# mythos-bio/mythos

Measured on AMD Instinct MI355X. Metric: MD steps/sec (and ns/day) per GPU, oxDNA2 12 kbp duplex, higher is better.
Workload: dtype f32; 1 GPU; oxDNA2 12000 bp duplex (24000 nt), Debye-Hueckel salt 0.5, Langevin dt 0.005, free space, 1 replica/GPU; half_charged_ends=True, replicas=1, repeats=1, warmup_steps_done=10405, precision=headline f32 (north_star: fp32 at 1e-3); the other precision: --full, full=False

## Files before the change

include/mythos_hip.h:

```cpp
#ifndef MYTHOS_HIP_H
#define MYTHOS_HIP_H

#include <stdint.h>

#ifdef __cplusplus
extern "C" {
#endif

typedef struct mythos_system mythos_system_t;
typedef struct mythos_sim mythos_sim_t;
typedef struct mythos_martini mythos_martini_t;
typedef struct mythos_martini_sim mythos_martini_sim_t;
typedef struct mythos_obs mythos_obs_t;
typedef void* mythos_stream_t;

enum mythos_status {
  MYTHOS_OK = 0,
  MYTHOS_ERR_INVALID_ARGUMENT = -1,
  MYTHOS_ERR_HIP = -2,
  MYTHOS_ERR_NO_DEVICE = -3,
  MYTHOS_ERR_NOT_READY = -4,
  MYTHOS_ERR_OVERFLOW = -5,
  MYTHOS_ERR_NUMERIC = -6
};
// ... 107 lines not shown
int mythos_langevin_set_option(mythos_sim_t* sim, int option, int64_t value);

int mythos_langevin_set_timing(mythos_sim_t* sim, int samples);
int mythos_langevin_last_kernel_ms(const mythos_sim_t* sim, double* kernel_ms, double* loop_ms_per_launch,
                                   int* launches, int* samples);

int mythos_langevin_last_recoveries(const mythos_sim_t* sim, int* recoveries);
int mythos_langevin_last_rebuilds(const mythos_sim_t* sim, int* scheduled);

int mythos_umbrella_check(int n, int n_rep, int model, int n_bonded, const int32_t* bonded, int n_ops, const int32_t* op_kind,
                          const int32_t* op_first, const int32_t* pairs, int n_pairs, const int32_t* iface_first,
                          const double* interfaces, const int32_t* table_shape, const double* table, int segment_steps);
int mythos_langevin_set_umbrella(mythos_sim_t* sim, int n_rep, int n_ops, const int32_t* op_kind, const int32_t* op_first,
                                 const int32_t* pairs, int n_pairs, const int32_t* iface_first, const double* interfaces,
                                 const int32_t* table_shape, const double* table, double hb_cutoff, int segment_steps);
int mythos_langevin_advance_umbrella(mythos_sim_t* sim, int n_segments, int sample_every, void* traj_center, void* traj_quat,
                                     void* prop_center, void* prop_quat, double* record, mythos_stream_t stream);
int mythos_langevin_umbrella_counts(mythos_sim_t* sim, int64_t* accepted, int64_t* decided);

int mythos_oxdna_read_trajectory(const char* path, int n, int max_frames, double* times, double* box, double* energies,
                                 double* frames, int* n_frames);

int mythos_oxdna_write_trajectory(const char* path, int n, int n_frames, const double* times, const double* box,
                                  const double* energies, const double* frames, int append);

enum mythos_debug_key {
  MYTHOS_DEBUG_CELL_BUCKET_CAP = 0,
  MYTHOS_DEBUG_ENERGY_LIST_CAP = 1,
  MYTHOS_DEBUG_MD_SEGMENT = 2,
  MYTHOS_DEBUG_MD_OVERFLOW_AT = 3,
  MYTHOS_DEBUG_MD_DENSE = 4,
  MYTHOS_DEBUG_MD_ITEMS_BIG = 5,
  MYTHOS_DEBUG_MD_LANES = 6,
  MYTHOS_DEBUG_KEYS = 7
};
int mythos_debug_set(int key, int64_t value);
int64_t mythos_debug_get(int key);

#define MYTHOS_MARTINI_N_TERMS 3
mythos_martini_t* mythos_martini_create(int n, const int32_t* types, int n_types, const double* sigma,
                                        const double* eps, int n_bonds, const int32_t* bonds, const double* bond_k,
                                        const double* bond_r0, int n_angles, const int32_t* angles,
                                        const double* angle_k, const double* angle_t0, int angle_kind, double r_cut,
                                        int dtype, int device);
void mythos_martini_destroy(mythos_martini_t* m);
int mythos_martini_set_params(mythos_martini_t* m, const double* sigma, const double* eps, const double* bond_k, const double* bond_r0,
                              const double* angle_k, const double* angle_t0);
int mythos_martini_energy(mythos_martini_t* m, const void* pos, const void* box, int n_frames, double* e_terms,
                          void* dU_dpos, mythos_stream_t stream);

int mythos_martini_param_grads(mythos_martini_t* m, const void* pos, const void* box, int n_frames, double* d_sigma,
                               double* d_eps, double* d_bond_k, double* d_bond_r0, double* d_angle_k,
                               double* d_angle_t0, mythos_stream_t stream);

int mythos_martini_set_charges(mythos_martini_t* m, const double* q, double epsilon_r, double epsilon_rf);
int mythos_martini_coulomb(mythos_martini_t* m, const void* pos, const void* box, int n_frames, double* e_coul,
                           void* dU_dpos, mythos_stream_t stream);

mythos_martini_sim_t* mythos_martini_langevin_create(mythos_martini_t* sys, double dt, double kT, double gamma,
                                                     const double* mass, uint64_t seed);
void mythos_martini_langevin_destroy(mythos_martini_sim_t* sim);
int mythos_martini_langevin_set_neighbor_policy(mythos_martini_sim_t* sim, double skin, int rebuild_every);
int mythos_martini_langevin_set_inner_list(mythos_martini_sim_t* sim, double margin, int every);
int mythos_martini_langevin_init_velocities(mythos_martini_sim_t* sim, void* vel, mythos_stream_t stream);
int mythos_martini_langevin_run(mythos_martini_sim_t* sim, void* pos, void* vel, const double* box, int n_steps,
                                int save_every, void* traj_pos, double* e_trace, mythos_stream_t stream);
int mythos_martini_langevin_load(mythos_martini_sim_t* sim, const void* pos, const void* vel, const double* box,
// ... 99 lines not shown
```

mythos_amd/_lib.py:

```python

from __future__ import annotations

import ctypes as C
import os
from pathlib import Path

import torch

_LIB_PATH = Path(__file__).resolve().parent / "lib" / "libmythos_hip.so"

c_int_p = C.POINTER(C.c_int32)
c_double_p = C.POINTER(C.c_double)
c_uint8_p = C.POINTER(C.c_uint8)


class MythosHipError(RuntimeError):
    """An error reported by libmythos_hip.so."""


_lib = None

V = C.c_void_p
_SIGS = {
    "mythos_version": (C.c_char_p, []),
# ... 139 lines not shown
            f"{path} not found: the HIP extension is not built (run __graft_entry__.build()). "
            "mythos_amd has no CPU fallback."
        )
    lib = C.CDLL(str(path))
    for name, (res, args) in _SIGS.items():
        fn = getattr(lib, name)
        fn.restype = res
        fn.argtypes = args
    _lib = lib
    return lib


DECLARED_SYMBOLS = tuple(_SIGS)


MEMBRANE_ROW = 7


def last_error() -> str:
    return load().mythos_last_error().decode()


def check(rc: int, what: str = "") -> None:
    if rc == 0:
        return
    msg = f"{what}: {last_error()} (status {rc})"
    if rc == -1:
        raise ValueError(msg)
    if rc == -6:
        raise FloatingPointError(msg)
    raise MythosHipError(msg)


DEBUG_KEYS = {"cell_bucket_cap": 0, "energy_list_cap": 1, "md_segment": 2, "md_overflow_at": 3, "md_dense": 4, "md_items_big": 5, "md_lanes": 6}


def debug_set(key: str, value: int) -> None:
    check(load().mythos_debug_set(DEBUG_KEYS[key], int(value)), f"debug_set({key})")


def debug_get(key: str) -> int:
    return int(load().mythos_debug_get(DEBUG_KEYS[key]))


_PARAM_NAMES: list[str] = []


def param_names() -> list[str]:
    if not _PARAM_NAMES:
        lib = load()
        _PARAM_NAMES.extend(lib.mythos_oxdna_param_name(i).decode() for i in range(lib.mythos_oxdna_param_count()))
    return list(_PARAM_NAMES)


def device_count() -> int:
    return int(load().mythos_device_count())


def ptr(t):
    if t is None:
        return None
    if hasattr(t, "data_ptr"):
        return C.c_void_p(t.data_ptr())
    return C.c_void_p(t.ctypes.data)


def stream(device) -> C.c_void_p:
# ... 41 lines not shown
```

mythos_amd/csrc/capi.hip:

```cpp
#include <atomic>
#include <cmath>
#include <cstring>
#include <memory>

#include "cell_list.h"
#include "observables.h"

namespace mythos {

static thread_local std::string g_last_error;

void set_error(const std::string& msg) { g_last_error = msg; }

int hip_fail(hipError_t e, const char* what) {
  g_last_error = std::string("HIP error: ") + hipGetErrorString(e) + " in " + what;
  return MYTHOS_ERR_HIP;
}

static std::atomic<long long> g_debug[MYTHOS_DEBUG_KEYS];

long long debug_value(int key) { return (key >= 0 && key < MYTHOS_DEBUG_KEYS) ? g_debug[key].load(std::memory_order_relaxed) : 0; }
void debug_clear(int key) {
  if (key >= 0 && key < MYTHOS_DEBUG_KEYS) g_debug[key].store(0, std::memory_order_relaxed);
}

static const char* const kParamNames[] = {
#define OXP(name) #name,
#include "oxdna_param_list.inc"
#undef OXP
};

}

using namespace mythos;

extern "C" {

const char* mythos_version(void) { return "mythos_amd 0.1 (gfx950)"; }

const char* mythos_last_error(void) { return g_last_error.c_str(); }

int mythos_device_count(void) {
  int n = 0;
  if (hipGetDeviceCount(&n) != hipSuccess) return 0;
  return n;
}

int mythos_debug_set(int key, int64_t value) {
  if (key < 0 || key >= MYTHOS_DEBUG_KEYS || value < 0) {
    set_error("mythos_debug_set: unknown key or negative value");
    return MYTHOS_ERR_INVALID_ARGUMENT;
  }
// ... 315 lines not shown
```

mythos_amd/csrc/langevin.hip:

```cpp
#include <algorithm>
#include <memory>
#include <vector>

#include "langevin_core.inc"
#include "point_force_checks.h"

namespace {
MdEntries md_entries_of(const mythos_sim* s) { return s->sys->dtype == MYTHOS_F32 ? md_entries<float>() : md_entries_f64(); }

ExtFieldView ext_point_part(const ExtFieldView& v) {
  ExtFieldView o;
  o.n_points = v.n_points;
  o.pt_kind = v.pt_kind, o.pt_particle = v.pt_particle, o.pt_ref = v.pt_ref, o.pt_flags = v.pt_flags, o.pt_param = v.pt_param;
  for (int a = 0; a < 3; ++a) o.box[a] = v.box[a];
  return o;
}

int ext_entries_merge(mythos_sim* s) {
  const std::vector<int>&ri = s->h_rst_index, &rf = s->h_rst_first, &rt = s->h_rst_term, &pp = s->h_pt_particle;
  ExtFieldView& v = s->rst;
  v.n_entries = v.n_points = 0;
  v.e_index = v.e_first = v.e_term = v.pt_first = nullptr;
  std::vector<int> e_index, e_first{0}, e_term, pt_first{0};
  size_t a = 0, b = 0;
// ... 37 lines not shown
  s->device = sys->device;
  s->dt = dt;
  s->kT = kT;
  s->gamma_t = gamma_t;
  s->gamma_r = gamma_r;
  s->mass = mass;
  for (int k = 0; k < 3; ++k) s->inertia[k] = inertia ? inertia[k] : 1.0;
  s->seed = seed;
  const size_t v4 = (sys->dtype == MYTHOS_F32 ? sizeof(float4) : sizeof(double4)) * (size_t)sys->n;
  bool ok = md_run_create(*s);
  for (int k = 0; k < 2; ++k)
    for (int a = 0; a < mythos_sim::kFrameArrays; ++a) ok = ok && s->frame[k][a].alloc(v4) == 0;
  ok = ok && s->keep_hi.alloc(v4) == 0 && s->keep_lo.alloc(v4) == 0 &&
       s->d_epart.alloc((size_t)((sys->n + 15) / 16) * kTraceWidth) == 0 && sys->reserve_refs() == 0;
  if (!ok) {
    set_error("mythos_langevin_create: device allocation failed");
    return nullptr;
  }
  return s.release();
}

void mythos_langevin_destroy(mythos_sim_t* s) { delete s; }

int mythos_langevin_set_neighbor_policy(mythos_sim_t* s, double r_cut, double skin, int every) {
  if (!s || (every > 0 && (!(r_cut > 0) || !(skin > 0)))) {
    set_error("mythos_langevin_set_neighbor_policy: invalid argument");
    return MYTHOS_ERR_INVALID_ARGUMENT;
  }
  s->r_cut = r_cut;
  s->skin = skin;
  s->rebuild_every = every;
  s->list_fitted = false;
  s->list_valid = false;
  return MYTHOS_OK;
}

int mythos_langevin_init_momenta(mythos_sim_t* s, void* p_lin, void* p_ang, mythos_stream_t stream) {
  if (!s || !p_lin || !p_ang) {
    set_error("mythos_langevin_init_momenta: invalid argument");
    return MYTHOS_ERR_INVALID_ARGUMENT;
  }
  MYTHOS_HIP_TRY(hipSetDevice(s->device));
  return md_entries_of(s).init_momenta(s, p_lin, p_ang, (hipStream_t)stream);
}

namespace {

int md_ready_state(mythos_sim_t* s, const char* who) {
  mythos_system* sys = s->sys;
  if (!sys->params_set) {
    set_error(std::string(who) + ": parameters must be set first");
    return MYTHOS_ERR_NOT_READY;
  }
  if (sys->model == 4 && !sys->types_set) {
    set_error(std::string(who) + ": an oxNA system needs its nucleotide types (mythos_oxdna_set_nucleotide_types)");
    return MYTHOS_ERR_NOT_READY;
  }
  MYTHOS_HIP_TRY(hipSetDevice(sys->device));
  return MYTHOS_OK;
}

int md_ready(mythos_sim_t* s, const char* who) {
  mythos_system* sys = s->sys;
  if (int rc = md_ready_state(s, who)) return rc;
  if (!sys->nbrs_set && s->rebuild_every <= 0) {
    set_error(std::string(who) + ": parameters and neighbours (or a neighbour policy) must be set first");
// ... 553 lines not shown
```

mythos_amd/csrc/langevin_core.inc:

```
#include <algorithm>
#include <cmath>
#include <type_traits>

#include <hip/hip_ext.h>

#ifndef MYTHOS_LEAN_MATH
#define MYTHOS_LEAN_MATH 1
#endif

#include "cell_list.h"
#include "chunk_order.h"
#include "md_driver.h"
#include "md_plan.h"
#include "oxdna_gather.h"
#include "philox.h"

#include "langevin_step.h"
#include "langevin_frame.h"
#include "ext_field.h"
#include "langevin_unfused.inc"

using namespace mythos;

namespace mythos {
// ... 126 lines not shown
                               (const int*)sim->d_flags.get(), (const int*)halt_words, k, stamp, sim->d_rst_stamp.get(), st);
    }
    auto launch = [&](auto save_tag, auto items_tag, auto pseq_tag, auto dense_tag, auto lanes_tag) {
      hipExtLaunchKernelGGL((md_step_kernel<R, MODEL, decltype(save_tag)::value, decltype(items_tag)::value, decltype(pseq_tag)::value,
                                            decltype(dense_tag)::value, decltype(lanes_tag)::value>),
                            dim3(plan.grid), dim3(kMdBlock), 0, st, row.ea, row.eb, 0,
                            Pdev, box, K, cut, n, fr[cur], fr[cur ^ 1], sys->list.d_rows.get(), sys->d_row_len.get(), row_close_of(sys),
                            sys->list.stride, sys->extra_bonds ? 1 : 0, kick_close, row.do_step, sim->seed, (uint64_t)(sim->step + k), ref,
                            ref_off, ref_a1, sim->d_flags.get(), tc, tq, sim->d_epart.get(), sim->d_chunk_order.get(), halt_words, k, 0,
                            plan.prio_on, pseq);
    };
    with_bool(save, [&](auto save_tag) {
      with_bool(sim->items_big, [&](auto big_tag) {
        constexpr bool SV = decltype(save_tag)::value;
        using Items = std::integral_constant<int, decltype(big_tag)::value ? md_items_big<R, SV>() : kMdItems>;
        with_bool(use_pseq, [&](auto pseq_tag) {
          using L8 = std::integral_constant<int, 8>;
          using L16 = std::integral_constant<int, 16>;
          constexpr bool dense_exists = sizeof(R) == 4 && !SV && !decltype(pseq_tag)::value && Items::value == kMdItems && MODEL <= 2;
          if (sim->lanes == 16) {
            launch(save_tag, Items{}, pseq_tag, std::false_type{}, L16{});
          } else if constexpr (dense_exists) {
            with_bool(plan.dense_grid, [&](auto dense_tag) { launch(save_tag, Items{}, pseq_tag, dense_tag, L8{}); });
          } else {
            launch(save_tag, Items{}, pseq_tag, std::false_type{}, L8{});
          }
        });
      });
    });
    if (save)
      hipLaunchKernelGGL(reduce_trace_kernel<kTraceWidth>, dim3(1), dim3(256), 0, st, sim->d_epart.get(), blocks,
                         e_trace + (size_t)row.sidx * kTraceWidth);
  };
  auto rebuild = [&](int buf) -> int {
    if ((++sim->builds & 63) == 0)
      if (int rc = update_chunk_order<R>(sim, fr[buf].p0, blocks, st)) return rc;
    return rows_build_device(sys, fr[buf].p0, true, sim->r_cut, sim->skin, fr[buf].p3, fr[buf].p1, true, st);
  };
  auto rebuild_until_fit = [&](int buf) -> int {
    return rows_build_until_fit(sys, fr[buf].p0, true, sim->r_cut, sim->skin, fr[buf].p3, fr[buf].p1, true, true, st);
  };
  auto on_abort = [&]() -> int {
    if (!sim->items_big) {
      sim->items_big = true;
      return 0;
    }
    set_error("mythos_langevin_run: more than " + std::to_string(md_items_big<R, false>()) + " (" + std::to_string(md_items_big<R, true>()) +
              " on steps that save energies)"
              " neighbours of one nucleotide are inside the range of an angular term (overlapping bases?)");
    return MYTHOS_ERR_OVERFLOW;
  };
  MdDrive d;
  d.who = "mythos_langevin_run";
  d.n_steps = n_steps, d.save_every = save_every, d.close = close;
  d.energy_rows = save_every > 0 && e_trace != nullptr;
  d.plain_rows = save_every > 0 && e_trace == nullptr && (traj_center != nullptr || traj_quat != nullptr);
  d.dynamic_list = dynamic_list;
  d.halt_words = halt_words;
  d.row_stride = &sys->list.stride;
  d.skin = sim->skin;
  d.st = st;
  return md_drive(*sim, d, launch_step, rebuild, rebuild_until_fit, on_abort);
}

template <typename R>
static int entry_load(mythos_sim* s, void* c, void* q, void* p, void* l, hipStream_t st) {
  if (s->unfused.active) return unfused_load<R>(s, (R*)c, (R*)q, (R*)p, (R*)l, st);
  return with_model(s->sys->model, [&](auto m) { return load_typed<R, decltype(m)::value>(s, (R*)c, (R*)q, (R*)p, (R*)l, st); });
}

template <typename R>
static int entry_advance(mythos_sim* s, int n_steps, int save_every, bool close, void* tc, void* tq, double* e_trace, hipStream_t st) {
// ... 71 lines not shown
```

mythos_amd/csrc/langevin_sim.h:

```cpp
#pragma once
#ifndef MYTHOS_UNFUSED_STATE_DEFINED
#error "langevin_sim.h needs UnfusedState: include langevin_unfused.inc (or langevin_core.inc), which defines it and then includes this file"
#endif
#include <cmath>
#include <vector>

#include "ext_field.h"
#include "langevin_step.h"
#include "md_driver.h"
#include "umbrella.h"

struct mythos_sim : mythos::MdRun {
  mythos_system* sys = nullptr;
  int device = 0;
  double dt = 0, kT = 0, gamma_t = 0, gamma_r = 0, mass = 1, inertia[3] = {1, 1, 1};
  double r_cut = 0, skin = 0;
  static constexpr int kFrameArrays = 8;
  mythos::DeviceBytes frame[2][kFrameArrays];
  int builds = 0;
  int list_epoch = 0;
  mythos::DeviceBytes keep_hi, keep_lo;
  bool keep_valid = false;
  bool items_big = false;
  int param_epoch = 0;
  int lanes = mythos::kMdG;
  mythos::DeviceBuf<int> d_chunk_order;
  mythos::DeviceBuf<unsigned long long> d_chunk_keys;
  mythos::DeviceBuf<double> d_epart;
  mythos::UnfusedState unfused;
  int ext_count = 0;
  mythos::DeviceBuf<int> d_ext_index;
  mythos::DeviceBytes d_ext_force;
  mythos::DeviceBuf<unsigned long long> d_ext_stamp;
  bool ext_stamp_stale = true;
  mythos::ExtFieldView rst;
  mythos::DeviceBuf<int> d_rst_t_index, d_rst_t_mask, d_rst_g_kind, d_rst_g_first, d_rst_g_member, d_rst_g_mask;
  mythos::DeviceBuf<int> d_rst_e_index, d_rst_e_first, d_rst_e_term;
  mythos::DeviceBuf<double> d_rst_t_k, d_rst_t_anchor, d_rst_g_vec, d_rst_g_target, d_rst_g_row;
  mythos::DeviceBuf<unsigned long long> d_rst_stamp;
  bool rst_stamp_stale = true;
  mythos::DeviceBuf<int> d_pt_first, d_pt_kind, d_pt_particle, d_pt_ref, d_pt_flags;
  mythos::DeviceBuf<double> d_pt_param;
  std::vector<int> h_rst_index, h_rst_first{0}, h_rst_term, h_pt_particle;
  bool pt_moving = false;
  mythos::UmbrellaState umb;
  mythos::DeviceBytes d_eval_p0, d_eval_mom, d_eval_ctl;
  mythos::DeviceBuf<double> d_eval_group_row;
  ~mythos_sim() { (void)hipSetDevice(device); }
};

namespace mythos {

template <typename R>
// ... 45 lines not shown
```

mythos_amd/csrc/mythos_internal.h:

```cpp
#pragma once
#include <hip/hip_runtime.h>

#include <algorithm>
#include <cmath>
#include <cstdint>
#include <string>
#include <type_traits>
#include <vector>

#include "../../include/mythos_hip.h"
#include "device_buf.h"
#include "oxdna_math.h"

namespace mythos {

long long debug_value(int key);
void debug_clear(int key);

constexpr int ROW_ROLE_Q = 1 << 30;
constexpr int ROW_INDEX_MASK = ROW_ROLE_Q - 1;
constexpr int ROW_BONDED_SLOTS = 4;

template <typename R>
struct BoxT {
// ... 13 lines not shown
  int cell_alloc_bucket_cap = 0;
  bool cell_sites = false;
  int cell_bucket_cap;
  int cell_phase = 0;
  explicit VerletRows(int bucket_cap) : cell_bucket_cap(bucket_cap) {}
};

}

struct mythos_obs;

struct mythos_system {
  int model = 0;
  int n = 0;
  int dtype = 0;
  int device = 0;
  int n_bonded = 0;
  bool has_box = false;
  double box[3] = {0, 0, 0};

  mythos::DeviceBuf<int> d_meta;

  mythos::VerletRows list{32};
  mythos::DeviceBuf<int> d_row_len;
  bool nbrs_set = false;
  int list_epoch = 0;
  int param_epoch = 0;
  std::vector<int> h_partners;
  bool extra_bonds = false;

  mythos::DeviceBytes d_ref_pos;
  mythos::DeviceBytes d_ref_off;
  mythos::DeviceBytes d_ref_a1;
  int reserve_refs() {
    const size_t v4 = (dtype == MYTHOS_F32 ? sizeof(float4) : sizeof(double4)) * (size_t)n;
    for (mythos::DeviceBytes* b : {&d_ref_pos, &d_ref_off, &d_ref_a1})
      if (int rc = b->grow(v4)) return rc;
    return 0;
  }

  bool params_set = false;
  mythos::OxParams<float> pf;
  mythos::OxParams<double> pd;
  std::vector<double> pd_sets;
  int param_sets() const { return model == 4 ? 3 : 1; }
  bool types_set = false;
  std::vector<int> h_meta;
  mythos::DeviceBuf<float> d_pf;
  mythos::DeviceBuf<double> d_pd;

  mythos::DeviceBytes d_ps_marg;
  mythos::DeviceBuf<int> d_ps_unit;
  mythos::DeviceBytes d_ps_bp;
  int pseq_terms = 0;
  int ps_n_bp = 0;
  double* ps_gmarg = nullptr;
  double* ps_gbp = nullptr;

  mythos::DeviceBuf<double> d_epart;
  mythos::DeviceBuf<double> d_pgpart;
  mythos::DeviceBuf<double> d_sweep_consts;
  mythos::DeviceBuf<double> d_sweep_part;
  std::vector<int> h_op_list;
  mythos::DeviceBuf<int> d_op_list;

  ~mythos_system() { (void)hipSetDevice(device); }
// ... 57 lines not shown
  return sys->param_sets() == 1 ? sys->pd.v : sys->pd_sets.data() + (size_t)k * OXP_COUNT;
}
inline double oxdna_param_max(const mythos_system* sys, int idx) {
  double m = oxdna_param_set(sys, 0)[idx];
  for (int k = 1; k < sys->param_sets(); ++k) m = std::max(m, oxdna_param_set(sys, k)[idx]);
  return m;
}

inline double oxdna_close_range(const mythos_system* sys) {
  double off_back = 0.0, off_base = 0.0, off_stack = 0.0;
  for (int k = 0; k < std::min(sys->param_sets(), 2); ++k) {
    const double* P = oxdna_param_set(sys, k);
    off_back = std::max(off_back, std::sqrt(P[GEO_BACK_A1] * P[GEO_BACK_A1] + (sys->model >= 2 ? P[GEO_BACK_A2] * P[GEO_BACK_A2] : 0.0)));
    off_base = std::max(off_base, std::fabs(P[GEO_BASE]));
    off_stack = std::max(off_stack, std::fabs(P[GEO_STACK]));
  }
  auto mx = [&](int idx) { return oxdna_param_max(sys, idx); };
  double rcom = std::max(mx(NEXC_BACK_BASE_RC), mx(NEXC_BASE_BACK_RC)) + off_back + off_base;
  rcom = std::max(rcom, mx(NEXC_BASE_RC) + 2 * off_base);
  rcom = std::max(rcom, std::max(mx(HYDR_RCHIGH), mx(CRST_RCHIGH)) + 2 * off_base);
  rcom = std::max(rcom, mx(CXST_RCHIGH) + 2 * off_stack);
  return rcom * (1.0 + 1e-6);
}

int oxdna_energy_launch(mythos_system* sys, const void* center, const void* quat, int n_frames, double* e_terms,
                        void* dU_dcenter, void* dU_dquat, double* dU_dparams, mythos_obs* obs, double* obs_out,
                        hipStream_t stream);
int rows_from_pairs(mythos_system* sys, const int32_t* pairs, int n_pairs);
int rows_build_device(mythos_system* sys, const void* center, bool center_is_vec4, double r_cut, double skin,
                      const void* backbone_offsets, const void* base_vectors, bool write_refs, hipStream_t stream);
int rows_build_until_fit(mythos_system* sys, const void* center, bool center_is_vec4, double r_cut, double skin,
                         const void* backbone_offsets, const void* base_vectors, bool write_refs, bool headroom,
                         hipStream_t stream);

}
```

mythos_amd/csrc/neighbors.hip:

```cpp
#include <algorithm>
#include <cmath>

#include "cell_list.h"
#include "oxdna_gather.h"

namespace mythos {

int rows_from_pairs(mythos_system* sys, const int32_t* pairs, int n_pairs) {
  const int n = sys->n;
  std::vector<int> count(n, 0);
  for (int k = 0; k < n_pairs; ++k) {
    const int i = pairs[2 * k], j = pairs[2 * k + 1];
    if (i < 0 || j < 0 || i >= n || j >= n || i == j) {
      set_error("set_neighbors: pair index out of range or i == j");
      return MYTHOS_ERR_INVALID_ARGUMENT;
    }
    ++count[i];
    ++count[j];
  }
  int mx = 0;
  for (int c : count) mx = std::max(mx, c);
  const int stride = ((mx + ROW_BONDED_SLOTS + 15) / 16) * 16;
  std::vector<int> rows((size_t)n * stride, -1), len(n, ROW_BONDED_SLOTS);
  for (int i = 0; i < n; ++i) {
    for (int k = 0; k < ROW_BONDED_SLOTS; ++k) rows[(size_t)i * stride + k] = sys->h_partners[(size_t)ROW_BONDED_SLOTS * i + k];
  }
  for (int k = 0; k < n_pairs; ++k) {
    const int i = pairs[2 * k], j = pairs[2 * k + 1];
    rows[(size_t)i * stride + len[i]++] = j;
    rows[(size_t)j * stride + len[j]++] = i | ROW_ROLE_Q;
  }
  if (int rc = rows_reserve(sys->list, n, stride)) return rc;
  MYTHOS_HIP_TRY(hipMemcpy(sys->list.d_rows.get(), rows.data(), rows.size() * sizeof(int), hipMemcpyHostToDevice));
  MYTHOS_HIP_TRY(hipMemcpy(sys->d_row_len.get(), len.data(), n * sizeof(int), hipMemcpyHostToDevice));
  MYTHOS_HIP_TRY(hipMemcpy(row_close_of(sys), len.data(), n * sizeof(int), hipMemcpyHostToDevice));
  sys->nbrs_set = true;
  return 0;
// ... 207 lines not shown
      if (k < kSegCap) s_far[k] = e;
    }
    out_c += __popc(mc);
    out_f += __popc(mf);
  }
  __builtin_amdgcn_wave_barrier();
  __builtin_amdgcn_fence(__ATOMIC_ACQ_REL, "wavefront");
  const int n_close = ROW_BONDED_SLOTS + out_c;
  int out = n_close + out_f;
  group_sort_to_row<G>(s_close, min(out_c, kSegCap), row + ROW_BONDED_SLOTS, row_stride - ROW_BONDED_SLOTS, l);
  if (n_close < row_stride) group_sort_to_row<G>(s_far, min(out_f, kSegCap), row + n_close, row_stride - n_close, l);
  if (l == 0) {
    row[0] = bp.x, row[1] = bp.y, row[2] = bp.z, row[3] = bp.w;
    if (out > row_stride) {
      atomicMax(overflow, out);
      out = row_stride;
    }
    row_len[i] = out;
    row_close[i] = min(n_close, out);
    if (ref_pos) {
      R* rp = ref_pos + 4 * (size_t)i;
      rp[0] = ci.x, rp[1] = ci.y, rp[2] = ci.z, rp[3] = VEC4 ? pos[S * i + 3] : R(0);
      if (sc.off) {
        R* ro = ref_off + 4 * (size_t)i;
        R* ra = ref_a1 + 4 * (size_t)i;
#pragma unroll
        for (int k = 0; k < 4; ++k) ro[k] = sc.off[4 * (size_t)i + k], ra[k] = sc.a1[4 * (size_t)i + k];
      }
    }
  }
}

template <typename R>
static int build_cells_typed(mythos_system* sys, const R* pos, bool vec4, double rl, double skin, const R* off,
                             const R* a1, bool write_refs, hipStream_t st) {
  R* ref_pos = write_refs ? (R*)sys->d_ref_pos.get() : nullptr;
  R* ref_off = write_refs ? (R*)sys->d_ref_off.get() : nullptr;
  R* ref_a1 = write_refs ? (R*)sys->d_ref_a1.get() : nullptr;
  const int n = sys->n;
  const double rcl = sys->params_set ? std::min(rl, oxdna_close_range(sys) + skin) : rl;
  int* d_close = row_close_of(sys);
  double rbb = rl;
  if (off && sys->params_set) {
    rbb = oxdna_param_max(sys, NEXC_BACKBONE_RC);
    if (sys->model >= 2) rbb = std::max(rbb, oxdna_param_max(sys, DH_RCUT));
    rbb = std::min(rl, rbb + skin);
  }
  if (!sys->params_set || !a1) off = nullptr;
  SiteCrit<R> sc{off, a1, R(rbb * rbb), R(0), R(0), R(0), R(0), R(0)};
  if (off) {
    auto mx = [&](int idx) { return oxdna_param_max(sys, idx); };
    const double* Pd = oxdna_param_set(sys, 0);
    const double* Pr = oxdna_param_set(sys, sys->param_sets() == 1 ? 0 : 1);
    const double slack_ba = std::fabs(Pd[GEO_BASE] - Pr[GEO_BASE]), slack_st = std::fabs(Pd[GEO_STACK] - Pr[GEO_STACK]);
    auto sq = [&](double r) { return R((r + skin) * (r + skin)); };
    sc.rbase2 = sq(std::max({mx(HYDR_RCHIGH), mx(CRST_RCHIGH), mx(NEXC_BASE_RC)}) + slack_ba);
    sc.rstack2 = sq(mx(CXST_RCHIGH) + slack_st);
    sc.rkb2 = sq(std::max(mx(NEXC_BACK_BASE_RC), mx(NEXC_BASE_BACK_RC)) + 0.5 * slack_ba);
    sc.g_ba = R(0.5 * (Pd[GEO_BASE] + Pr[GEO_BASE]));
    sc.g_st = R(0.5 * (Pd[GEO_STACK] + Pr[GEO_STACK]));
  }
  VerletRows& L = sys->list;
  CellGrid<R> g;
  const bool cells = cell_grid(g, n, rl, sys->has_box ? sys->box : nullptr);
  const int blocks_ap = (n * 64 + 255) / 256;
  int* d_partners = sys->d_row_len.get() + n;
  const BoxT<R> box = make_box<R>(sys);
  if (!cells) {
    if (vec4)
      hipLaunchKernelGGL((build_rows_allpairs_kernel<R, true>), dim3(blocks_ap), dim3(256), 0, st, n, pos, box,
                         R(rl * rl), R(rcl * rcl), sc, d_partners, L.d_rows.get(), sys->d_row_len.get(), d_close, L.stride, L.d_overflow.get());
    else
      hipLaunchKernelGGL((build_rows_allpairs_kernel<R, false>), dim3(blocks_ap), dim3(256), 0, st, n, pos, box,
                         R(rl * rl), R(rcl * rcl), sc, d_partners, L.d_rows.get(), sys->d_row_len.get(), d_close, L.stride, L.d_overflow.get());
    if (write_refs && vec4) {
      const size_t bytes = (size_t)n * 4 * sizeof(R);
      MYTHOS_HIP_TRY(hipMemcpyAsync(ref_pos, pos, bytes, hipMemcpyDeviceToDevice, st));
      if (sc.off) {
        MYTHOS_HIP_TRY(hipMemcpyAsync(ref_off, sc.off, bytes, hipMemcpyDeviceToDevice, st));
        MYTHOS_HIP_TRY(hipMemcpyAsync(ref_a1, sc.a1, bytes, hipMemcpyDeviceToDevice, st));
      }
    }
    return 0;
  }
  const bool sites = sc.off != nullptr && vec4;
  CellBins bins;
  if (int rc = cell_table<R>(L, next_pow2(2 * n), sites, st, bins)) return rc;
  const size_t site_stride = sites ? (size_t)bins.H * bins.cap : 0;
  if (vec4)
    cell_bins_build<R, true>(n, pos, g, bins, L.d_overflow.get(), false, st, sc.off, sc.a1);
  else
    cell_bins_build<R, false>(n, pos, g, bins, L.d_overflow.get(), false, st);
  constexpr int kPerBlock = 256 / kRowG;
  const int wb = (n + kPerBlock - 1) / kPerBlock;
  const size_t far_lds = (size_t)kPerBlock * 2 * L.stride * sizeof(int);
  if (vec4)
    hipLaunchKernelGGL((build_rows_cells_kernel<R, true, kRowG>), dim3(wb), dim3(256), far_lds, st, n, pos, box, g, R(rl * rl),
                       R(rcl * rcl), sc, d_partners, bins.cnt_cur, (const typename CellPlace<R>::type*)bins.place, bins.cap, bins.spill, bins.H, site_stride, L.d_rows.get(), sys->d_row_len.get(), d_close, L.stride,
                       L.d_overflow.get(), ref_pos, ref_off, ref_a1);
  else
    hipLaunchKernelGGL((build_rows_cells_kernel<R, false, kRowG>), dim3(wb), dim3(256), far_lds, st, n, pos, box, g, R(rl * rl),
                       R(rcl * rcl), sc, d_partners, bins.cnt_cur, (const typename CellPlace<R>::type*)bins.place, bins.cap, bins.spill, bins.H, site_stride, L.d_rows.get(), sys->d_row_len.get(), d_close, L.stride,
                       L.d_overflow.get(), ref_pos, ref_off, ref_a1);
  return 0;
}

int rows_build_device(mythos_system* sys, const void* center, bool center_is_vec4, double r_cut, double skin,
                      const void* backbone_offsets, const void* base_vectors, bool write_refs, hipStream_t stream) {
  if (sys->list.stride == 0)
    if (int rc = rows_reserve(sys->list, sys->n, 64)) return rc;
  const double rl = r_cut + skin;
  int rc;
  if (sys->dtype == MYTHOS_F32)
    rc = build_cells_typed<float>(sys, (const float*)center, center_is_vec4, rl, skin, (const float*)backbone_offsets, (const float*)base_vectors, write_refs, stream);
  else
    rc = build_cells_typed<double>(sys, (const double*)center, center_is_vec4, rl, skin, (const double*)backbone_offsets, (const double*)base_vectors, write_refs, stream);
  if (rc) return rc;
  MYTHOS_HIP_TRY(hipGetLastError());
  sys->nbrs_set = true;
  return 0;
}

int rows_build_until_fit(mythos_system* sys, const void* center, bool center_is_vec4, double r_cut, double skin,
                         const void* backbone_offsets, const void* base_vectors, bool write_refs, bool headroom,
                         hipStream_t stream) {
  return list_build_until_fit(
      sys->list, sys->n,
      [&] { return rows_build_device(sys, center, center_is_vec4, r_cut, skin, backbone_offsets, base_vectors, write_refs, stream); },
      headroom, "neighbour build", stream);
}

}
```

Before: 70780 steps/s.

## Build neighbour rows by filtering a wider cached candidate list

Adds a two-level neighbour list. A wide candidate list (cutoff plus an extra margin) is built with the cell grid once every several rebuilds, and ordinary Verlet rebuilds just filter those candidates with a new kernel instead of rebinning and scanning cells each time. A displacement check against the candidate reference positions flags any row the candidates can no longer vouch for, and this falls back through the overflow path. The intent is to cut the cost of frequent list rebuilds, in exchange for extra memory, a larger candidate scan per filter pass, and more complex state handling. It is on by default through a debug key that defaults to 1.

```diff
diff --git a/include/mythos_hip.h b/include/mythos_hip.h
--- a/include/mythos_hip.h
+++ b/include/mythos_hip.h
@@ -163,7 +163,10 @@
   MYTHOS_DEBUG_MD_DENSE = 4,
   MYTHOS_DEBUG_MD_ITEMS_BIG = 5,
   MYTHOS_DEBUG_MD_LANES = 6,
-  MYTHOS_DEBUG_KEYS = 7
+  MYTHOS_DEBUG_ROWS_FILTER = 7,
+  MYTHOS_DEBUG_ROWS_CAND_EVERY = 8,
+  MYTHOS_DEBUG_ROWS_CAND_MARGIN = 9,
+  MYTHOS_DEBUG_KEYS = 10
 };
 int mythos_debug_set(int key, int64_t value);
 int64_t mythos_debug_get(int key);
diff --git a/mythos_amd/_lib.py b/mythos_amd/_lib.py
--- a/mythos_amd/_lib.py
+++ b/mythos_amd/_lib.py
@@ -195,7 +195,8 @@
     raise MythosHipError(msg)
 
 
-DEBUG_KEYS = {"cell_bucket_cap": 0, "energy_list_cap": 1, "md_segment": 2, "md_overflow_at": 3, "md_dense": 4, "md_items_big": 5, "md_lanes": 6}
+DEBUG_KEYS = {"cell_bucket_cap": 0, "energy_list_cap": 1, "md_segment": 2, "md_overflow_at": 3, "md_dense": 4, "md_items_big": 5, "md_lanes": 6,
+              "rows_filter": 7, "rows_cand_every": 8, "rows_cand_margin": 9}
 
 
 def debug_set(key: str, value: int) -> None:
diff --git a/mythos_amd/csrc/capi.hip b/mythos_amd/csrc/capi.hip
--- a/mythos_amd/csrc/capi.hip
+++ b/mythos_amd/csrc/capi.hip
@@ -18,6 +18,7 @@
 }
 
 static std::atomic<long long> g_debug[MYTHOS_DEBUG_KEYS];
+static const bool g_debug_defaults = (g_debug[MYTHOS_DEBUG_ROWS_FILTER].store(1, std::memory_order_relaxed), true);
 
 long long debug_value(int key) { return (key >= 0 && key < MYTHOS_DEBUG_KEYS) ? g_debug[key].load(std::memory_order_relaxed) : 0; }
 void debug_clear(int key) {
diff --git a/mythos_amd/csrc/langevin.hip b/mythos_amd/csrc/langevin.hip
--- a/mythos_amd/csrc/langevin.hip
+++ b/mythos_amd/csrc/langevin.hip
@@ -93,6 +93,7 @@
   s->rebuild_every = every;
   s->list_fitted = false;
   s->list_valid = false;
+  s->sys->cand_unfit = false;
   return MYTHOS_OK;
 }
 
diff --git a/mythos_amd/csrc/langevin_core.inc b/mythos_amd/csrc/langevin_core.inc
--- a/mythos_amd/csrc/langevin_core.inc
+++ b/mythos_amd/csrc/langevin_core.inc
@@ -182,12 +182,34 @@
       hipLaunchKernelGGL(reduce_trace_kernel<kTraceWidth>, dim3(1), dim3(256), 0, st, sim->d_epart.get(), blocks,
                          e_trace + (size_t)row.sidx * kTraceWidth);
   };
+  const int cand_every = cand_every_for(debug_value(MYTHOS_DEBUG_ROWS_CAND_EVERY));
+  const double cand_margin = cand_margin_for(debug_value(MYTHOS_DEBUG_ROWS_CAND_MARGIN));
+  const int cand_margin_milli = (int)std::lround(1e3 * cand_margin);
+  bool filter_rows = dynamic_list && debug_value(MYTHOS_DEBUG_ROWS_FILTER) != 0 && !sys->cand_unfit &&
+                     rows_filter_applies(sys, sim->r_cut, sim->skin, cand_margin);
   auto rebuild = [&](int buf) -> int {
     if ((++sim->builds & 63) == 0)
       if (int rc = update_chunk_order<R>(sim, fr[buf].p0, blocks, st)) return rc;
-    return rows_build_device(sys, fr[buf].p0, true, sim->r_cut, sim->skin, fr[buf].p3, fr[buf].p1, true, st);
+    if (!filter_rows) {
+      sim->cand = cand_none();
+      return rows_build_device(sys, fr[buf].p0, true, sim->r_cut, sim->skin, fr[buf].p3, fr[buf].p1, true, st);
+    }
+    const bool wide = cand_rebuild_is_wide(sim->cand, sim->list_valid, cand_every, cand_margin_milli);
+    if (wide) {
+      sim->cand = cand_none();
+      if (int rc = rows_wide_build_device(sys, fr[buf].p0, sim->r_cut, sim->skin, cand_margin, st)) return rc;
+    }
+    sim->cand = cand_after(wide, sim->cand, cand_margin_milli);
+    return rows_filter_device(sys, fr[buf].p0, fr[buf].p3, fr[buf].p1, sim->r_cut, sim->skin, cand_margin, st);
   };
   auto rebuild_until_fit = [&](int buf) -> int {
+    sim->cand = cand_none();
+    if (filter_rows) {
+      const int rc = rows_filter_until_fit(sys, fr[buf].p0, fr[buf].p3, fr[buf].p1, sim->r_cut, sim->skin, cand_margin, st);
+      if (rc == MYTHOS_OK) sim->cand = cand_after(true, sim->cand, cand_margin_milli);
+      if (!sys->cand_unfit) return rc;
+      filter_rows = false;
+    }
     return rows_build_until_fit(sys, fr[buf].p0, true, sim->r_cut, sim->skin, fr[buf].p3, fr[buf].p1, true, true, st);
   };
   auto on_abort = [&]() -> int {
diff --git a/mythos_amd/csrc/langevin_sim.h b/mythos_amd/csrc/langevin_sim.h
--- a/mythos_amd/csrc/langevin_sim.h
+++ b/mythos_amd/csrc/langevin_sim.h
@@ -8,6 +8,7 @@
 #include "ext_field.h"
 #include "langevin_step.h"
 #include "md_driver.h"
+#include "row_filter_plan.h"
 #include "umbrella.h"
 
 struct mythos_sim : mythos::MdRun {
@@ -19,6 +20,7 @@
   mythos::DeviceBytes frame[2][kFrameArrays];
   int builds = 0;
   int list_epoch = 0;
+  mythos::CandState cand;
   mythos::DeviceBytes keep_hi, keep_lo;
   bool keep_valid = false;
   bool items_big = false;
diff --git a/mythos_amd/csrc/mythos_internal.h b/mythos_amd/csrc/mythos_internal.h
--- a/mythos_amd/csrc/mythos_internal.h
+++ b/mythos_amd/csrc/mythos_internal.h
@@ -69,6 +69,10 @@
   mythos::DeviceBytes d_ref_pos;
   mythos::DeviceBytes d_ref_off;
   mythos::DeviceBytes d_ref_a1;
+  mythos::VerletRows cand{32};
+  mythos::DeviceBuf<int> d_cand_len;
+  mythos::DeviceBytes d_cand_ref;
+  bool cand_unfit = false;
   int reserve_refs() {
     const size_t v4 = (dtype == MYTHOS_F32 ? sizeof(float4) : sizeof(double4)) * (size_t)n;
     for (mythos::DeviceBytes* b : {&d_ref_pos, &d_ref_off, &d_ref_a1})
@@ -192,5 +196,11 @@
 int rows_build_until_fit(mythos_system* sys, const void* center, bool center_is_vec4, double r_cut, double skin,
                          const void* backbone_offsets, const void* base_vectors, bool write_refs, bool headroom,
                          hipStream_t stream);
-
-}
+bool rows_filter_applies(const mythos_system* sys, double r_cut, double skin, double margin);
+int rows_wide_build_device(mythos_system* sys, const void* p0, double r_cut, double skin, double margin, hipStream_t stream);
+int rows_filter_device(mythos_system* sys, const void* p0, const void* p3, const void* p1, double r_cut, double skin, double margin,
+                       hipStream_t stream);
+int rows_filter_until_fit(mythos_system* sys, const void* p0, const void* p3, const void* p1, double r_cut, double skin, double margin,
+                          hipStream_t stream);
+
+}
diff --git a/mythos_amd/csrc/neighbors.hip b/mythos_amd/csrc/neighbors.hip
--- a/mythos_amd/csrc/neighbors.hip
+++ b/mythos_amd/csrc/neighbors.hip
@@ -3,6 +3,7 @@
 
 #include "cell_list.h"
 #include "oxdna_gather.h"
+#include "row_filter_plan.h"
 
 namespace mythos {
 
@@ -276,14 +277,7 @@
 }
 
 template <typename R>
-static int build_cells_typed(mythos_system* sys, const R* pos, bool vec4, double rl, double skin, const R* off,
-                             const R* a1, bool write_refs, hipStream_t st) {
-  R* ref_pos = write_refs ? (R*)sys->d_ref_pos.get() : nullptr;
-  R* ref_off = write_refs ? (R*)sys->d_ref_off.get() : nullptr;
-  R* ref_a1 = write_refs ? (R*)sys->d_ref_a1.get() : nullptr;
-  const int n = sys->n;
-  const double rcl = sys->params_set ? std::min(rl, oxdna_close_range(sys) + skin) : rl;
-  int* d_close = row_close_of(sys);
+static SiteCrit<R> site_crit_for(const mythos_system* sys, double rl, double skin, const R* off, const R* a1) {
   double rbb = rl;
   if (off && sys->params_set) {
     rbb = oxdna_param_max(sys, NEXC_BACKBONE_RC);
@@ -304,9 +298,27 @@
     sc.g_ba = R(0.5 * (Pd[GEO_BASE] + Pr[GEO_BASE]));
     sc.g_st = R(0.5 * (Pd[GEO_STACK] + Pr[GEO_STACK]));
   }
-  VerletRows& L = sys->list;
+  return sc;
+}
+
+template <typename R>
+static int build_cells_typed(mythos_system* sys, const R* pos, bool vec4, double rl, double skin, const R* off,
+                             const R* a1, bool write_refs, hipStream_t st, bool wide = false) {
+  R* ref_pos = write_refs ? (R*)(wide ? sys->d_cand_ref.get() : sys->d_ref_pos.get()) : nullptr;
+  R* ref_off = write_refs ? (R*)sys->d_ref_off.get() : nullptr;
+  R* ref_a1 = write_refs ? (R*)sys->d_ref_a1.get() : nullptr;
+  const int n = sys->n;
+  const double rcl = (sys->params_set && !wide) ? std::min(rl, oxdna_close_range(sys) + skin) : rl;
+  int* d_len = wide ? sys->d_cand_len.get() : sys->d_row_len.get();
+  int* d_close = wide ? d_len + n : row_close_of(sys);
+  const SiteCrit<R> sc = site_crit_for<R>(sys, rl, skin, off, a1);
+  VerletRows& L = wide ? sys->cand : sys->list;
   CellGrid<R> g;
   const bool cells = cell_grid(g, n, rl, sys->has_box ? sys->box : nullptr);
+  if (wide && !cells) {
+    set_error("candidate build: the system does not take the cell builder");
+    return MYTHOS_ERR_INVALID_ARGUMENT;
+  }
   const int blocks_ap = (n * 64 + 255) / 256;
   int* d_partners = sys->d_row_len.get() + n;
   const BoxT<R> box = make_box<R>(sys);
@@ -340,13 +352,186 @@
   const size_t far_lds = (size_t)kPerBlock * 2 * L.stride * sizeof(int);
   if (vec4)
     hipLaunchKernelGGL((build_rows_cells_kernel<R, true, kRowG>), dim3(wb), dim3(256), far_lds, st, n, pos, box, g, R(rl * rl),
-                       R(rcl * rcl), sc, d_partners, bins.cnt_cur, (const typename CellPlace<R>::type*)bins.place, bins.cap, bins.spill, bins.H, site_stride, L.d_rows.get(), sys->d_row_len.get(), d_close, L.stride,
+                       R(rcl * rcl), sc, d_partners, bins.cnt_cur, (const typename CellPlace<R>::type*)bins.place, bins.cap, bins.spill, bins.H, site_stride, L.d_rows.get(), d_len, d_close, L.stride,
                        L.d_overflow.get(), ref_pos, ref_off, ref_a1);
   else
     hipLaunchKernelGGL((build_rows_cells_kernel<R, false, kRowG>), dim3(wb), dim3(256), far_lds, st, n, pos, box, g, R(rl * rl),
-                       R(rcl * rcl), sc, d_partners, bins.cnt_cur, (const typename CellPlace<R>::type*)bins.place, bins.cap, bins.spill, bins.H, site_stride, L.d_rows.get(), sys->d_row_len.get(), d_close, L.stride,
+                       R(rcl * rcl), sc, d_partners, bins.cnt_cur, (const typename CellPlace<R>::type*)bins.place, bins.cap, bins.spill, bins.H, site_stride, L.d_rows.get(), d_len, d_close, L.stride,
                        L.d_overflow.get(), ref_pos, ref_off, ref_a1);
   return 0;
+}
+
+constexpr int kFilterBatch = 4;
+constexpr int kRowsUnvouched = 1;
+
+template <typename R, int G>
+__global__ __launch_bounds__(256) void filter_rows_kernel(int n, const typename Vec4T<R>::type* __restrict__ p0,
+                                                          const typename Vec4T<R>::type* __restrict__ p3,
+                                                          const typename Vec4T<R>::type* __restrict__ p1, const BoxT<R> box,
+                                                          R rc2, R rcl2, const SiteCrit<R> sc,
+                                                          const int* __restrict__ partners,
+                                                          const int* __restrict__ cand_rows, const int* __restrict__ cand_len,
+                                                          int cand_stride,
+                                                          const typename Vec4T<R>::type* __restrict__ cand_ref, R stale2,
+                                                          const int* __restrict__ cand_overflow, int* __restrict__ rows,
+                                                          int* __restrict__ row_len, int* __restrict__ row_close,
+                                                          int row_stride, int* __restrict__ overflow,
+                                                          typename Vec4T<R>::type* __restrict__ ref_pos,
+                                                          typename Vec4T<R>::type* __restrict__ ref_off,
+                                                          typename Vec4T<R>::type* __restrict__ ref_a1) {
+  using V4 = typename Vec4T<R>::type;
+  constexpr int NG = 256 / G;
+  extern __shared__ int s_far_all[];
+  const int grp = threadIdx.x / G, l = threadIdx.x % G;
+  const int gshift = (threadIdx.x & 63) & ~(G - 1);
+  const int i = blockIdx.x * NG + grp;
+  if (i >= n) return;
+  int* s_far = s_far_all + (size_t)grp * cand_stride;
+  const V4 c4 = p0[i], o4 = p3[i], a4 = p1[i], r4 = cand_ref[i];
+  const int ncand = min(cand_len[i], cand_stride) - ROW_BONDED_SLOTS;
+  const int* crow = cand_rows + (size_t)i * cand_stride + ROW_BONDED_SLOTS;
+  const V3<R> ci{c4.x, c4.y, c4.z};
+  const R oi[3] = {o4.x, o4.y, o4.z}, ai[3] = {a4.x, a4.y, a4.z};
+  int* row = rows + (size_t)i * row_stride;
+  int out_c = 0, out_f = 0;
+  constexpr unsigned int kGroupMask = (G == 32) ? 0xffffffffu : ((1u << G) - 1u);
+  const unsigned int below = (1u << l) - 1u;
+  for (int t0 = 0; t0 < ncand; t0 += kFilterBatch * G) {
+    int e[kFilterBatch];
+    V4 cj[kFilterBatch], oj4[kFilterBatch], aj4[kFilterBatch];
+#pragma unroll
+    for (int b = 0; b < kFilterBatch; ++b) {
+      const int t = t0 + b * G + l;
+      e[b] = (t < ncand) ? crow[t] : -1;
+    }
+#pragma unroll
+    for (int b = 0; b < kFilterBatch; ++b) {
+      const int j = (e[b] >= 0) ? (e[b] & ROW_INDEX_MASK) : i;
+      cj[b] = p0[j], oj4[b] = p3[j], aj4[b] = p1[j];
+    }
+#pragma unroll
+    for (int b = 0; b < kFilterBatch; ++b) {
+      if (t0 + b * G >= ncand) break;
+      bool hit_c = false, hit_f = false;
+      if (e[b] >= 0) {
+        const R oj[3] = {oj4[b].x, oj4[b].y, oj4[b].z}, aj[3] = {aj4[b].x, aj4[b].y, aj4[b].z};
+        V3<R> d{cj[b].x - ci.x, cj[b].y - ci.y, cj[b].z - ci.z};
+        d = min_image(d, box);
+        const R r2 = dot(d, d);
+        if (r2 < rc2) {
+          hit_c = r2 < rcl2 && site_close_v(sc, ai, oi, aj, oj, d);
+          hit_f = !hit_c && far_in_range_v(sc, oi, oj, d);
+        }
+      }
+      const unsigned int mc = (unsigned int)(__ballot(hit_c) >> gshift) & kGroupMask;
+      const unsigned int mf = (unsigned int)(__ballot(hit_f) >> gshift) & kGroupMask;
+      if (hit_c) {
+        const int k = ROW_BONDED_SLOTS + out_c + __popc(mc & below);
+        if (k < row_stride) row[k] = e[b];
+      }
+      if (hit_f) s_far[out_f + __popc(mf & below)] = e[b];
+      out_c += __popc(mc);
+      out_f += __popc(mf);
+    }
+  }
+  __builtin_amdgcn_wave_barrier();
+  __builtin_amdgcn_fence(__ATOMIC_ACQ_REL, "wavefront");
+  const int n_close = ROW_BONDED_SLOTS + out_c;
+  int out = n_close + out_f;
+  for (int k = l; k < out_f; k += G)
+    if (n_close + k < row_stride) row[n_close + k] = s_far[k];
+  if (l == 0) {
+    const int* bq = partners + (size_t)ROW_BONDED_SLOTS * i;
+    row[0] = bq[0], row[1] = bq[1], row[2] = bq[2], row[3] = bq[3];
+    if (out > row_stride) {
+      atomicMax(overflow, out);
+      out = row_stride;
+    }
+    row_len[i] = out;
+    row_close[i] = min(n_close, out);
+    V4 rp = c4;
+    ref_pos[i] = rp, ref_off[i] = o4, ref_a1[i] = a4;
+    V3<R> dr{ci.x - r4.x, ci.y - r4.y, ci.z - r4.z};
+    dr = min_image(dr, box);
+    bool unvouched = !(dot(dr, dr) <= stale2);
+    if (i == 0) unvouched = unvouched || (cand_overflow[0] | cand_overflow[1]) != 0;
+    if (unvouched) atomicMax(overflow, kRowsUnvouched);
+  }
+}
+
+bool rows_filter_applies(const mythos_system* sys, double r_cut, double skin, double margin) {
+  CellGrid<double> g;
+  return sys->params_set && cell_grid(g, sys->n, r_cut + skin + margin, sys->has_box ? sys->box : nullptr) &&
+         cell_grid(g, sys->n, r_cut + skin, sys->has_box ? sys->box : nullptr);
+}
+
+static int cand_reserve(mythos_system* sys) {
+  const int n = sys->n;
+  if (!sys->cand.d_overflow) {
+    if (int rc = sys->cand.d_overflow.alloc(kOverflowWords)) return rc;
+    MYTHOS_HIP_TRY(hipMemset(sys->cand.d_overflow.get(), 0, kOverflowWords * sizeof(int)));
+  }
+  if (!sys->d_cand_len)
+    if (int rc = sys->d_cand_len.alloc(2 * (size_t)n)) return rc;
+  if (int rc = sys->d_cand_ref.grow((sys->dtype == MYTHOS_F32 ? sizeof(float4) : sizeof(double4)) * (size_t)n)) return rc;
+  if (sys->cand.stride == 0)
+    if (int rc = rows_reserve(sys->cand, n, 96)) return rc;
+  return 0;
+}
+
+int rows_wide_build_device(mythos_system* sys, const void* p0, double r_cut, double skin, double margin, hipStream_t stream) {
+  if (int rc = cand_reserve(sys)) return rc;
+  const double rl = r_cut + skin + margin;
+  const int rc = with_real(sys->dtype, [&](auto real) {
+    using R = decltype(real);
+    return build_cells_typed<R>(sys, (const R*)p0, true, rl, skin + margin, nullptr, nullptr, true, stream, true);
+  });
+  if (rc) return rc;
+  MYTHOS_HIP_TRY(hipGetLastError());
+  return 0;
+}
+
+int rows_filter_device(mythos_system* sys, const void* p0, const void* p3, const void* p1, double r_cut, double skin, double margin,
+                       hipStream_t stream) {
+  if (sys->list.stride == 0)
+    if (int rc = rows_reserve(sys->list, sys->n, 64)) return rc;
+  const int n = sys->n;
+  const double rl = r_cut + skin;
+  const double rcl = std::min(rl, oxdna_close_range(sys) + skin);
+  constexpr int kPerBlock = 256 / kRowG;
+  const VerletRows& C = sys->cand;
+  VerletRows& L = sys->list;
+  with_real(sys->dtype, [&](auto real) {
+    using R = decltype(real);
+    using V4 = typename Vec4T<R>::type;
+    const SiteCrit<R> sc = site_crit_for<R>(sys, rl, skin, (const R*)p3, (const R*)p1);
+    hipLaunchKernelGGL((filter_rows_kernel<R, kRowG>), dim3((n + kPerBlock - 1) / kPerBlock), dim3(256),
+                       (size_t)kPerBlock * C.stride * sizeof(int), stream, n, (const V4*)p0, (const V4*)p3, (const V4*)p1, make_box<R>(sys),
+                       R(rl * rl), R(rcl * rcl), sc, (const int*)(sys->d_row_len.get() + n), (const int*)C.d_rows.get(),
+                       (const int*)sys->d_cand_len.get(), C.stride, (const V4*)sys->d_cand_ref.get(), R(cand_stale_sq(margin)),
+                       (const int*)C.d_overflow.get(), L.d_rows.get(), sys->d_row_len.get(), row_close_of(sys), L.stride,
+                       L.d_overflow.get(), (V4*)sys->d_ref_pos.get(), (V4*)sys->d_ref_off.get(), (V4*)sys->d_ref_a1.get());
+  });
+  MYTHOS_HIP_TRY(hipGetLastError());
+  sys->nbrs_set = true;
+  return 0;
+}
+
+int rows_filter_until_fit(mythos_system* sys, const void* p0, const void* p3, const void* p1, double r_cut, double skin, double margin,
+                          hipStream_t stream) {
+  if (int rc = cand_reserve(sys)) return rc;
+  constexpr int kCandStrideMax = 384;
+  auto wide = [&]() -> int {
+    if (sys->cand.stride > kCandStrideMax) {
+      sys->cand_unfit = true;
+      set_error("candidate build: more than " + std::to_string(kCandStrideMax) + " candidates in a row");
+      return MYTHOS_ERR_OVERFLOW;
+    }
+    return rows_wide_build_device(sys, p0, r_cut, skin, margin, stream);
+  };
+  if (int rc = list_build_until_fit(sys->cand, sys->n, wide, true, "candidate build", stream)) return rc;
+  return list_build_until_fit(
+      sys->list, sys->n, [&] { return rows_filter_device(sys, p0, p3, p1, r_cut, skin, margin, stream); }, true, "neighbour build", stream);
 }
 
 int rows_build_device(mythos_system* sys, const void* center, bool center_is_vec4, double r_cut, double skin,
diff --git a/mythos_amd/csrc/row_filter_plan.h b/mythos_amd/csrc/row_filter_plan.h
--- /dev/null
+++ b/mythos_amd/csrc/row_filter_plan.h
@@ -0,0 +1,31 @@
+#pragma once
+
+namespace mythos {
+
+constexpr int kCandEvery = 8;
+constexpr int kCandMarginMilli = 2000;
+
+inline int cand_every_for(long long debug_every) { return debug_every > 0 ? (int)(debug_every > 1 << 20 ? 1 << 20 : debug_every) : kCandEvery; }
+inline double cand_margin_for(long long debug_margin_milli) { return 1e-3 * double(debug_margin_milli > 0 ? debug_margin_milli : kCandMarginMilli); }
+
+inline double cand_stale_sq(double margin) {
+  const double h = 0.5 * margin * (1.0 - 1.0 / 512.0);
+  return h * h;
+}
+
+struct CandState {
+  int age = -1;
+  int margin_milli = 0;
+};
+
+inline bool cand_rebuild_is_wide(const CandState& c, bool list_valid, int every, int margin_milli) {
+  return !list_valid || c.age < 0 || c.margin_milli != margin_milli || c.age >= every;
+}
+
+inline CandState cand_after(bool wide, const CandState& c, int margin_milli) {
+  return wide ? CandState{1, margin_milli} : CandState{c.age + 1, c.margin_milli};
+}
+
+inline CandState cand_none() { return CandState{}; }
+
+}
```

New measurement: 72020 steps/s, median of 6. 1.7% higher.
